# rst-tu-dortmund/teb_local_planner

Hardware: AMD Instinct MI355X
Metric: TEB LM iterations/sec (whole node) (higher is better)
Workload: dtype f64; 1 GPU; C4: 256 candidate TEBs/GPU x 200 poses at the start (teb_autosize on, the reference default: 193..287 poses, mean 234, after the step), 500 point obstacles (50 dynamic), diff-drive, point footprint, TebConfig defaults, 4 outer x 5 inner; tebs_per_gpu=256, tebs_total=256, poses=200, pose_capacity=288, tebs_ok=256, obstacles=500, jacobian_mode=analytic (closed form), exchange=none (single GPU), binary_hash=10be306ab42698fd, binary_variant_defines=

## Files before the change

include/teb_amd.h:

```cpp
#ifndef TEB_AMD_H_
#define TEB_AMD_H_

#include <stdint.h>

#ifdef __cplusplus
extern "C" {
#endif

#define TEB_AMD_ABI_VERSION 3
#define TEB_AMD_MAX_POSES 944

enum {
  TEB_AMD_OK = 0,
  TEB_AMD_ERR_INVALID_ARG = 1,
  TEB_AMD_ERR_NO_DEVICE = 2,
  TEB_AMD_ERR_HIP = 3,
  TEB_AMD_ERR_CAPACITY = 4,
  TEB_AMD_ERR_UNSUPPORTED = 5
};

enum {
  TEB_AMD_TEB_OK = 0,
  TEB_AMD_TEB_FAILED = 1,
  TEB_AMD_TEB_NONFINITE = 2
// ... 147 lines not shown
       TEB_AMD_LAYOUT_BAND_HBM = 3 };
enum { TEB_AMD_HSIG3D_AUTO = 0, TEB_AMD_HSIG3D_WIDE = 1, TEB_AMD_HSIG3D_SMALL = 2 };
typedef struct teb_amd_options {
  int32_t struct_size;
  int32_t layout;
  int32_t fixed_layout;
  int32_t band_ldlt;
  int32_t generic_distance_path;
  int32_t hsig3d_kernel;
  int32_t no_near_cache;
  int32_t multi_cu;
  int32_t multi_cu_timeout_us;
  int32_t speculative_trials;
  int32_t generic_config_path;
  int32_t compile_for_config;
  int32_t reserved[4];
} teb_amd_options_t;
void teb_amd_options_default(teb_amd_options_t* opt);

int  teb_amd_create(const teb_amd_config_t* cfg, int32_t max_tebs, int32_t max_poses,
                    int32_t max_obstacles, int32_t max_obstacle_vertices, int32_t max_via_points,
                    int32_t device, void* stream, teb_amd_handle_t** out);
int  teb_amd_create_ex(const teb_amd_config_t* cfg, int32_t max_tebs, int32_t max_poses,
                       int32_t max_obstacles, int32_t max_obstacle_vertices, int32_t max_via_points,
                       int32_t device, void* stream, const teb_amd_options_t* options, teb_amd_handle_t** out);
void teb_amd_destroy(teb_amd_handle_t* h);
int  teb_amd_set_config(teb_amd_handle_t* h, const teb_amd_config_t* cfg);

int  teb_amd_set_obstacles(teb_amd_handle_t* h, const teb_amd_obstacles_t* obst);
int  teb_amd_set_via_points(teb_amd_handle_t* h, int32_t count, const double* x, const double* y);

// ... 124 lines not shown
```

include/teb_amd_debug.h:

```cpp
#ifndef TEB_AMD_DEBUG_H_
#define TEB_AMD_DEBUG_H_
#include "teb_amd.h"
#ifdef __cplusplus
extern "C" {
#endif

int teb_amd_sizeof_config(void);
int teb_amd_sizeof_obstacles(void);
int teb_amd_sizeof_teb_batch(void);
int teb_amd_sizeof_results(void);
int teb_amd_sizeof_options(void);

int teb_amd_debug_linearize(teb_amd_handle_t* h, int32_t b, double weight_multiplier, double* H_dense,
                            double* bvec, double* chi2, int32_t* assoc_pose, int32_t* assoc_obst,
                            int32_t assoc_cap, int32_t* assoc_count);

int teb_amd_debug_distance(teb_amd_handle_t* h, int32_t nq, const int32_t* obst_index, const double* x,
                           const double* y, const double* theta, const int32_t* spatio_temporal,
                           const double* t, double* dist, double* grad);

int teb_amd_debug_profile(teb_amd_handle_t* h, double* cycles8);
int teb_amd_debug_profile_bands(teb_amd_handle_t* h, double* cycles_per_band);

int teb_amd_debug_stream(teb_amd_handle_t* h, int64_t n_doubles, int32_t repeats);
// ... 10 lines not shown
int teb_amd_debug_last_config_profile(teb_amd_handle_t* h, int32_t* defaults_profile);
int teb_amd_debug_last_instantiation(teb_amd_handle_t* h, int32_t* solver, int32_t* jacobian_mode, int32_t* scene_kind);
int teb_amd_debug_rtc_stats(int32_t* ready, int32_t* compiling, int32_t* failed, double* last_compile_seconds, char* last_error, int32_t capacity);
int teb_amd_debug_rtc_join(void);
int teb_amd_debug_rtc_compile(uint64_t flag_values, int32_t solver, int32_t jacobian_mode, int32_t scene_kind, int64_t* code_bytes);
int teb_amd_debug_rtc_cache(int32_t* embedded, int32_t* disk_hits, int32_t* disk_writes, char* cache_dir, int32_t capacity);

int teb_amd_debug_build_info(char* kernel_hash, int32_t kernel_hash_capacity, char* source_hash, int32_t source_hash_capacity, char* variant_defines,
                             int32_t defines_capacity, int32_t* threads_per_workgroup);

#define TEB_AMD_PHASE_LOG_SLOTS 9
int teb_amd_set_phase_log(teb_amd_handle_t* h, int32_t enable);
int teb_amd_get_phase_log(teb_amd_handle_t* h, double* cycles, int32_t capacity_bands, int32_t* bands);

int teb_amd_debug_assoc_overflow(teb_amd_handle_t* h, int32_t* flags);

#ifdef __cplusplus
}
#endif
#endif
```

teb_local_planner_amd/_abi.py:

```python
import ctypes as C

import numpy as np

MAX_FOOTPRINT_VERTICES = 64

OK, ERR_INVALID_ARG, ERR_NO_DEVICE, ERR_HIP, ERR_CAPACITY, ERR_UNSUPPORTED = range(6)
MAX_POSES = 944
TEB_OK, TEB_FAILED, TEB_NONFINITE = range(3)
FOOTPRINT_POINT, FOOTPRINT_CIRCULAR, FOOTPRINT_TWO_CIRCLES, FOOTPRINT_LINE, FOOTPRINT_POLYGON = range(5)
OBST_POINT, OBST_CIRCULAR, OBST_LINE, OBST_PILL, OBST_POLYGON = range(5)
ROT_LEFT, ROT_NONE, ROT_RIGHT = range(3)
JACOBIAN_ANALYTIC, JACOBIAN_G2O_NUMERIC = range(2)

c_i32 = C.c_int32
c_f64 = C.c_double
p_i32 = C.POINTER(C.c_int32)
p_f64 = C.POINTER(C.c_double)


class Config(C.Structure):
    _fields_ = [
        ("teb_autosize", c_i32), ("dt_ref", c_f64), ("dt_hysteresis", c_f64),
        ("min_samples", c_i32), ("max_samples", c_i32), ("exact_arc_length", c_i32),
        ("via_points_ordered", c_i32),
# ... 54 lines not shown
        ("max_number_classes", c_i32), ("max_number_plans_in_current_class", c_i32), ("h_signature_prescaler", c_f64),
        ("h_signature_threshold", c_f64), ("allow_init_with_backwards_motion", c_i32), ("delete_detours_backwards", c_i32),
        ("detours_orientation_tolerance", c_f64), ("length_start_orientation_vector", c_f64),
        ("max_ratio_detours_duration_best_duration", c_f64), ("global_plan_overwrite_orientation", c_i32),
        ("viapoints_all_candidates", c_i32),
    ]


LAYOUT_AUTO, LAYOUT_BLOCKS_LDS, LAYOUT_BAND_LDS, LAYOUT_BAND_HBM = 0, 1, 2, 3
HSIG3D_AUTO, HSIG3D_WIDE, HSIG3D_SMALL = 0, 1, 2


class Options(C.Structure):
    _fields_ = [("struct_size", c_i32), ("layout", c_i32), ("fixed_layout", c_i32), ("band_ldlt", c_i32),
                ("generic_distance_path", c_i32), ("hsig3d_kernel", c_i32), ("no_near_cache", c_i32), ("multi_cu", c_i32),
                ("multi_cu_timeout_us", c_i32), ("speculative_trials", c_i32), ("generic_config_path", c_i32), ("compile_for_config", c_i32), ("reserved", c_i32 * 4)]

    def __init__(self, layout=LAYOUT_AUTO, fixed_layout=False, band_ldlt=False, generic_distance_path=False, hsig3d_kernel=HSIG3D_AUTO,
                 no_near_cache=False, multi_cu=0, multi_cu_timeout_us=0, speculative_trials=0, generic_config_path=False, compile_for_config=0):
        super().__init__()
        self.struct_size = C.sizeof(Options)
        self.layout = {"auto": LAYOUT_AUTO, "cr": LAYOUT_BLOCKS_LDS, "band": LAYOUT_BAND_LDS, "bandg": LAYOUT_BAND_HBM}.get(layout, layout)
        self.fixed_layout = int(fixed_layout)
        self.band_ldlt = int(band_ldlt)
        self.generic_distance_path = int(generic_distance_path)
        self.hsig3d_kernel = {"auto": HSIG3D_AUTO, "wide": HSIG3D_WIDE, "small": HSIG3D_SMALL}.get(hsig3d_kernel, hsig3d_kernel)
        self.no_near_cache = int(no_near_cache)
        self.multi_cu = int(multi_cu)
        self.multi_cu_timeout_us = int(multi_cu_timeout_us)
        self.speculative_trials = int(speculative_trials)
        self.generic_config_path = int(generic_config_path)
        self.compile_for_config = int(compile_for_config)


class Results(C.Structure):
    _fields_ = [
        ("status", p_i32), ("lm_iterations", p_i32), ("lm_trials", p_i32), ("chi2", p_f64),
        ("cost", p_f64), ("lambda_", p_f64),
    ]


def _ptr(a, ty):
    if a is None:
        return C.cast(None, C.POINTER(ty))
    return a.ctypes.data_as(C.POINTER(ty))


# ... 191 lines not shown
```

teb_local_planner_amd/csrc/teb_amd.hip:

```cpp
#include <hip/hip_runtime.h>

#include <chrono>
#include <cmath>
#include <cstdio>
#include <unistd.h>
#include <cstdlib>
#include <algorithm>
#include <cstring>
#include <limits>
#include <string>
#include <random>
#include <vector>

#include "../../include/teb_amd.h"
#include "../../include/teb_amd_debug.h"
#define TEB_AMD_MAIN_TU
#include "teb_kernel.hpp"
#include "teb_opt_launch.hpp"
#include "teb_fleet.hpp"
#include "teb_strip.hpp"
#include "teb_hsig.hpp"
#include "teb_graph.hpp"
#include "teb_comm.hpp"
#include "teb_rtc.hpp"
// ... 686 lines not shown
  const size_t assoc_bytes = sizeof(int) * (size_t)max_tebs * max_poses * (size_t)(max_obstacles > 0 ? max_obstacles : 1);
  if (assoc_bytes > ((size_t)64 << 30)) return fail(TEB_AMD_ERR_CAPACITY, "association table would exceed 64 GiB");

  teb_amd_handle* h = new teb_amd_handle();
  h->device = device;
  h->cfg = *cfg;
  h->opt = opt;
  h->max_tebs = max_tebs; h->stride = max_poses; h->max_obst = max_obstacles; h->max_verts = max_obstacle_vertices;
  h->max_via = max_via_points;
  h->lds_bytes = lds;
  h->solver = solver; h->solver_created = solver;
  h->lds_limit = lds_limit;
  h->num_cus = prop.multiProcessorCount;
  h->plan = make_lds_plan(max_poses, solver, 0, h->lds_limit);
  h->hmat_stride = std::max(hbm_scratch_doubles(max_poses, SOLVER_BAND), hbm_scratch_doubles(max_poses, solver));
  h->hmat_stride = (h->hmat_stride + 1) & ~(size_t)1;
  h->band_ldlt = opt.band_ldlt != 0;
  if (solver == SOLVER_BANDG) h->band_ldlt = 0;
  if (stream) { h->stream = reinterpret_cast<hipStream_t>(stream); h->own_stream = false; }
  else {
    if (hipStreamCreateWithFlags(&h->stream, hipStreamNonBlocking) != hipSuccess) { delete h; return fail(TEB_AMD_ERR_HIP, "hipStreamCreate failed"); }
    h->own_stream = true;
  }
  const size_t BS = (size_t)max_tebs * max_poses;
  const size_t Mo = max_obstacles > 0 ? max_obstacles : 1;
  bool ok = true;
  auto A = [&](hipError_t e) { if (e != hipSuccess) ok = false; };
  A(h->o_type.alloc(Mo)); A(h->o_dyn.alloc(Mo)); A(h->o_voff.alloc(Mo + 1)); A(h->o_static.alloc(Mo)); A(h->o_dynidx.alloc(Mo));
  A(h->o_list.alloc(5 * (size_t)Mo));
  A(h->o_ax.alloc(Mo)); A(h->o_ay.alloc(Mo)); A(h->o_bx.alloc(Mo)); A(h->o_by.alloc(Mo)); A(h->o_rad.alloc(Mo));
  A(h->o_vx.alloc(Mo)); A(h->o_vy.alloc(Mo)); A(h->o_cx.alloc(Mo)); A(h->o_cy.alloc(Mo)); A(h->o_brad.alloc(Mo));
  A(h->o_pvx.alloc(max_obstacle_vertices)); A(h->o_pvy.alloc(max_obstacle_vertices));
  A(h->viax.alloc(max_via_points)); A(h->viay.alloc(max_via_points));
  A(h->n.alloc(max_tebs)); A(h->has_vs.alloc(max_tebs)); A(h->has_vg.alloc(max_tebs)); A(h->rotdir.alloc(max_tebs));
  A(h->via_en.alloc(max_tebs)); A(h->status.alloc(max_tebs)); A(h->optimized.alloc(max_tebs)); A(h->iters.alloc(max_tebs)); A(h->last_iters.alloc(max_tebs)); A(h->trials.alloc(max_tebs));
  A(h->assoc_cnt.alloc(BS)); A(h->assoc.alloc(BS * Mo)); A(h->assoc_ovf.alloc(max_tebs)); A(h->legacy_idx.alloc((size_t)max_tebs * Mo));
  A(h->via_pose.alloc((size_t)max_tebs * (max_via_points > 0 ? max_via_points : 1)));
  A(h->x.alloc(BS)); A(h->y.alloc(BS)); A(h->th.alloc(BS)); A(h->dt.alloc(BS));
  A(h->vs.alloc(3 * (size_t)max_tebs)); A(h->vg.alloc(3 * (size_t)max_tebs));
  A(h->chi2.alloc(max_tebs)); A(h->cost.alloc(max_tebs)); A(h->lambda.alloc(max_tebs));
  A(h->Hbackup.alloc((size_t)max_tebs * h->hmat_stride));
  A(h->clk.alloc(4));
  h->hband_stride = solver == SOLVER_BANDG ? (((size_t)hbo(4 * max_poses) + 2 + 1) & ~(size_t)1) : 0;
  A(h->Hband.alloc((size_t)max_tebs * h->hband_stride));
  A(h->snap_n.alloc(max_tebs)); A(h->snap_x.alloc(BS)); A(h->snap_y.alloc(BS)); A(h->snap_th.alloc(BS)); A(h->snap_dt.alloc(BS));
  A(h->dbg_H.alloc((size_t)4 * max_poses * kBand)); A(h->dbg_b.alloc((size_t)4 * max_poses)); A(h->dbg_chi2.alloc(4));
  A(h->sel_cost.alloc(2)); A(h->sel_idx.alloc(1)); A(h->err_flag.alloc(1));
  A(h->pack_dev.alloc(kPackMaxDoubles));
  if (ok && hipHostMalloc(reinterpret_cast<void**>(&h->pack_host), kPackMaxDoubles * sizeof(double), hipHostMallocDefault) != hipSuccess) h->pack_host = nullptr;
  A(h->stage_x.alloc((size_t)max_poses + 2)); A(h->stage_y.alloc((size_t)max_poses + 2)); A(h->stage_yaw.alloc((size_t)max_poses + 2));
  A(h->out_cmd.alloc(4 * (size_t)max_tebs)); A(h->out_prof.alloc((size_t)max_tebs * (max_poses + 1) * 3)); A(h->out_traj.alloc(BS * 7));
  A(h->hsig.alloc((size_t)max_tebs * (Mo > 2 ? Mo : 2))); A(h->hs_pre.alloc(Mo)); A(h->hs_pim.alloc(Mo)); A(h->hs_pex.alloc(Mo));
  if (ok && hipEventCreate(&h->ev0) != hipSuccess) ok = false;
  if (ok && hipEventCreate(&h->ev1) != hipSuccess) ok = false;
  for (int sv : {SOLVER_BAND, SOLVER_CR, SOLVER_BANDG})
    for (int jm : {TEB_AMD_JACOBIAN_ANALYTIC, TEB_AMD_JACOBIAN_G2O_NUMERIC})
// ... 569 lines not shown
#ifndef TEB_AMD_HAS_FLEET_UNITS
    return fail(TEB_AMD_ERR_UNSUPPORTED, "fleet launches exist in the product library only; this one is the variant built with [" TEB_AMD_VARIANT_DEFINES "]");
#else
    if (h->cfg.jacobian_mode != TEB_AMD_JACOBIAN_ANALYTIC)
      return fail(TEB_AMD_ERR_INVALID_ARG, "fleet launches need jacobian_mode TEB_AMD_JACOBIAN_ANALYTIC");
    for (int b = 0; b < h->B; ++b)
      if (h->fleet.band_scene[b] >= h->fleet.n_scenes) {
        char buf[160];
        std::snprintf(buf, sizeof buf, "band %d maps to scene %d, but %d scenes are set (teb_amd_set_band_scenes)", b, h->fleet.band_scene[b], h->fleet.n_scenes);
        return fail(TEB_AMD_ERR_INVALID_ARG, buf);
      }
#endif
  }
  OptArgs a;
  std::memset(&a, 0, sizeof a);
  a.inner = inner; a.outer = outer; a.compute_cost = compute_cost; a.no_near_cache = h->opt.no_near_cache != 0; a.band_ldlt = (fleet ? h->fleet.solver : h->solver) == SOLVER_BANDG ? 0 : h->band_ldlt; a.Hband = h->Hband.p; a.hband_stride = h->hband_stride;
  a.obst_scale = obst_cost_scale; a.via_scale = viapoint_cost_scale; a.alt_time = alternative_time_cost;
  if (h->iter_log_on) { a.iter_log = h->iter_log.p; a.iter_log_cap = TEB_AMD_ITERATION_LOG_ROWS; }
  if (h->phase_log_on) a.phase_log = h->phase_log.p;
#ifdef TEB_PROFILE
  a.dbg_H = h->dbg_H.p;
#endif
  h->last_inner = inner;
  return launch(h, a);
}

int teb_amd_set_iteration_log(teb_amd_handle_t* h, int32_t enable) {
  int rc = check_handle(h);
  if (rc) return rc;
  if (enable && !h->iter_log.p) {
    const size_t count = (size_t)h->max_tebs * TEB_AMD_ITERATION_LOG_ROWS * 4;
// ... 1386 lines not shown
    int S = kThreads * kPoseIterBandHbm;
    while (S > 2 && lds_bytes_for(S, SOLVER_BANDG, h->lds_limit) > h->lds_limit) --S;
    *max_poses_supported = S;
  }
  return TEB_AMD_OK;
}

int teb_amd_debug_linearize(teb_amd_handle_t* h, int32_t b, double weight_multiplier, double* H_dense, double* bvec,
                            double* chi2, int32_t* assoc_pose, int32_t* assoc_obst, int32_t assoc_cap, int32_t* assoc_count) {
  int rc = check_handle(h);
  if (rc) return rc;
  if ((rc = refuse_in_fleet_mode(h, "teb_amd_debug_linearize"))) return rc;
  if (b < 0 || b >= h->B) return fail(TEB_AMD_ERR_INVALID_ARG, "TEB index out of range");
  OptArgs a;
  std::memset(&a, 0, sizeof a);
  a.inner = 1; a.outer = 1; a.no_near_cache = h->opt.no_near_cache != 0; a.debug_linearize = 1; a.debug_weight_multiplier = weight_multiplier; a.band_ldlt = h->solver == SOLVER_BANDG ? 0 : h->band_ldlt; a.Hband = h->Hband.p; a.hband_stride = h->hband_stride;
  a.dbg_H = h->dbg_H.p; a.dbg_b = h->dbg_b.p; a.dbg_chi2 = h->dbg_chi2.p;
  SceneDev sc = scene_of(h);
  BatchDev bt = batch_of(h);
  const size_t so = (size_t)b * h->stride;
  bt.B = 1;
  bt.n += b; bt.x += so; bt.y += so; bt.th += so; bt.dt += so;
  bt.has_vs += b; bt.vs += 3 * b; bt.has_vg += b; bt.vg += 3 * b; bt.rotdir += b; bt.via_en += b;
  bt.status += b; bt.iters += b; bt.last_iters += b; bt.trials += b; bt.chi2 += b; bt.cost += b; bt.lambda += b;
  bt.assoc_cnt += so; bt.assoc += (size_t)b * bt.assoc_cap * h->stride; bt.assoc_overflow += b;
  bt.via_pose += (size_t)b * bt.via_cap; bt.Hbackup += (size_t)b * h->hmat_stride;
  int sv_i[3]; double sv_d[3];
  HIPCHK(hipMemcpy(&sv_i[0], h->status.p + b, sizeof(int), hipMemcpyDeviceToHost));
  HIPCHK(hipMemcpy(&sv_i[1], h->iters.p + b, sizeof(int), hipMemcpyDeviceToHost));
  HIPCHK(hipMemcpy(&sv_i[2], h->trials.p + b, sizeof(int), hipMemcpyDeviceToHost));
  HIPCHK(hipMemcpy(&sv_d[0], h->chi2.p + b, sizeof(double), hipMemcpyDeviceToHost));
// ... 273 lines not shown
  int rc = check_handle(h);
  if (rc) return rc;
  if (!defaults_profile) return fail(TEB_AMD_ERR_INVALID_ARG, "null output");
  *defaults_profile = h->last_defaults_profile;
  return TEB_AMD_OK;
}

int teb_amd_debug_mcu_flags(teb_amd_handle_t* h, int32_t flags) {
  int rc = check_handle(h);
  if (rc) return rc;
  h->mcu_debug_flags = flags;
  return TEB_AMD_OK;
}


int teb_amd_debug_assoc_overflow(teb_amd_handle_t* h, int32_t* flags) {
  int rc = check_handle(h);
  if (rc) return rc;
  HIPCHK(hipMemcpy(flags, h->assoc_ovf.p, h->B * sizeof(int), hipMemcpyDeviceToHost));
  return TEB_AMD_OK;
}

}
```

teb_local_planner_amd/csrc/teb_device.hpp:

```cpp
#pragma once
#include <hip/hip_runtime.h>
#include <stdint.h>

#include "../../include/teb_amd.h"

#define TEB_PF_ALL(X)                                                                                                              \
  X(EXACT_ARC) X(COST_EXPONENT) X(NEW_ASSOCIATION) X(DYNAMIC_EDGES) X(VIA_POINTS) X(NONHOLONOMIC_VELOCITY) X(VELOCITY_EDGES)      \
  X(ACCELERATION_EDGES) X(NONHOLONOMIC_ACCELERATION) X(TIME_OPTIMAL) X(SHORTEST_PATH) X(VELOCITY_OBSTACLE_RATIO) X(RADIUS_FREE)   \
  X(DEBUG_LINEARIZE) X(BAND_LDLT) X(INFLATED) X(NO_NEAR_CACHE) X(DIVERGENCE_DETECTION) X(KIN_DIFF_DRIVE) X(KIN_EDGES)
#define TEB_PF_EXPR_EXACT_ARC (c.exact_arc_length)
#define TEB_PF_DFLT_EXACT_ARC false
#define TEB_PF_EXPR_COST_EXPONENT (c.obstacle_cost_exponent != 1.0 && c.min_obstacle_dist > 0.0)
#define TEB_PF_DFLT_COST_EXPONENT false
#define TEB_PF_EXPR_NEW_ASSOCIATION (!c.legacy_obstacle_association)
#define TEB_PF_DFLT_NEW_ASSOCIATION true
#define TEB_PF_EXPR_DYNAMIC_EDGES (c.include_dynamic_obstacles && c.weight_obstacle != 0)
#define TEB_PF_DFLT_DYNAMIC_EDGES true
#define TEB_PF_HOST_DYNAMIC_EDGES (c.weight_obstacle != 0)
#define TEB_PF_EXPR_VIA_POINTS (sc.nvia > 0 && c.weight_viapoint != 0)
#define TEB_PF_DFLT_VIA_POINTS false
#define TEB_PF_WIDE_VIA_POINTS 1
#define TEB_PF_EXPR_NONHOLONOMIC_VELOCITY (c.max_vel_y == 0)
#define TEB_PF_DFLT_NONHOLONOMIC_VELOCITY true
#define TEB_PF_WIDE_NONHOLONOMIC_VELOCITY 1
// ... 208 lines not shown
  size_t hmat_stride;
  long long* clk;
};

struct OptArgs {
  int inner, outer, compute_cost;
  double obst_scale, via_scale;
  int alt_time;
  double* Hband;
  size_t hband_stride;
  int band_ldlt;
  int no_near_cache;
  double* iter_log;
  int iter_log_cap;
  int debug_linearize;
  double debug_weight_multiplier;
  double* dbg_H;
  double* dbg_b;
  double* dbg_chi2;
  double* phase_log;
};
constexpr int kPhaseLogSlots = 9;

}
```

teb_local_planner_amd/csrc/teb_kernel.hpp:

```cpp
#pragma once
#include "teb_edges.hpp"
#include "teb_multicu.hpp"
#include "teb_autoresize_chain.hpp"

namespace tebamd {

#ifdef TEB_PROFILE
#define PROF_DECL long long prof_t0 = 0, prof_wg_t0 = clock64(), prof_acc[8] = {0, 0, 0, 0, 0, 0, 0, 0};
#define PROF_START() prof_t0 = clock64()
#define PROF_END(k) prof_acc[k] += clock64() - prof_t0
#else
#define PROF_DECL const bool plog_ = args.phase_log != nullptr; long long* const plog_acc_ = reinterpret_cast<long long*>(l.red + 40); \
  if (plog_ && threadIdx.x == 0) { for (int q_ = 0; q_ < 9; ++q_) plog_acc_[q_] = 0; plog_acc_[9] = clock64(); }
#define PROF_START() do { if (plog_ && threadIdx.x == 0) plog_acc_[8] = clock64(); } while (0)
#define PROF_END(k) do { if (plog_ && threadIdx.x == 0) plog_acc_[k] += clock64() - plog_acc_[8]; } while (0)
#endif

#ifdef TEB_PROFILE
__device__ long long g_ev_prof[8];
#define EVP_DECL long long evp_t0 = clock64(), evp_t1;
#define EVP(k) do { __builtin_amdgcn_sched_barrier(0); asm volatile("s_waitcnt vmcnt(0) lgkmcnt(0)" ::: "memory"); evp_t1 = clock64(); __builtin_amdgcn_sched_barrier(0); if (blockIdx.x == 0 && threadIdx.x == 1) g_ev_prof[k] += evp_t1 - evp_t0; evp_t0 = evp_t1; } while (0)
__device__ unsigned long long g_assoc_stats[4];
__device__ unsigned long long g_ar_steps[4];
__device__ unsigned long long g_near_recomputed, g_near_queries;
// ... 31 lines not shown

__host__ __device__ inline int nb_for(int S) { return (4 * S + 7) / 8; }
constexpr size_t kLdsHeadroomBytes = 1024;
__host__ __device__ inline size_t hmat_doubles(int S, int solver) {
  if (solver == SOLVER_BANDG) return (size_t)6 * S + 256;
  if (solver == SOLVER_CR) return (size_t)nb_for(S) * (2 * kBlk + 8);
  const size_t band = (size_t)hbo(4 * S), compact = (size_t)((nb_for(S) + 1) / 2) * (2 * kBlk + 8) + 14;
  return ((band > compact ? band : compact) + 1) & ~(size_t)1;
}
__host__ __device__ inline size_t hbm_scratch_doubles(int S, int solver) {
  const size_t nb = (size_t)nb_for(S);
  const size_t blocks = nb * (2 * kBlk + 8);
  const size_t own = hmat_doubles(S, solver);
  return own > blocks ? own : blocks;
}
__host__ inline LdsPlan make_lds_plan(int S, int solver, int ob_entries, size_t lds_limit_bytes) {
  LdsPlan p;
  p.S = S; p.solver = solver;
  int o = 0;
  p.off_state = o; o += 7 * S;
  o = (o + 1) & ~1;
  int hm = (int)hmat_doubles(S, solver);
  if (solver == SOLVER_BANDG) {
    const long long room = (long long)(lds_limit_bytes / 8) - (o + 8LL * S + 16 + 96 + 5LL * (ob_entries > 0 ? ob_entries : 0)), want = 64LL * 2 * kBlk;
    const long long extra = (room < want ? room : want) & ~1LL;
    if (extra > hm) hm = (int)extra;
  }
  p.off_H = o; o += hm;
  p.off_b = o; o += 4 * S + 8;
  p.off_dx = o; o += 4 * S + 8;
// ... 93 lines not shown
  return bi;
}

struct TebCtx {
  int b, n;
  int has_vs, has_vg, rotdir, via_en;
  double vs[3], vg[3];
  double w_obst;
  bool inflated;
  const int* assoc_cnt;
  const int* assoc;
  const int* via_pose;
  int stride;
  int assoc_cap;
  McuView mcu;
};

__device__ __forceinline__ double footprint_bound_radius(const teb_amd_config_t& c) {
  double frad = 0;
  if (c.footprint_type == TEB_AMD_FOOTPRINT_CIRCULAR) frad = c.footprint_radius;
  else if (c.footprint_type == TEB_AMD_FOOTPRINT_TWO_CIRCLES)
    frad = fmax(fabs(c.footprint_front_offset) + c.footprint_front_radius, fabs(c.footprint_rear_offset) + c.footprint_rear_radius);
  else if (c.footprint_type == TEB_AMD_FOOTPRINT_LINE || c.footprint_type == TEB_AMD_FOOTPRINT_POLYGON)
    for (int v = 0; v < c.footprint_n_vertices; ++v) frad = fmax(frad, sqrt(c.footprint_vx[v] * c.footprint_vx[v] + c.footprint_vy[v] * c.footprint_vy[v]));
  return frad;
}
__device__ __forceinline__ double distance_lower_bound(const SceneDev& sc, int oi, double x, double y, double frad) {
  const double bx = sc.cx[oi] - x, by = sc.cy[oi] - y;
  const double lbd = sqrt(bx * bx + by * by) - sc.brad[oi] - frad;
  return lbd - 1e-9 * (fabs(lbd) + sc.brad[oi] + frad + 1.0);
// ... 60 lines not shown
  if (uncached || __any(!(ddx * ddx + ddy * ddy <= lim * lim))) {
    int d_lo, d_hi;
    dyn_chunk(sc, sl, nsl, d_lo, d_hi);
    mask = dyn_near_mask<MODE>(c, sc, l, i, d_lo, d_lo + 64 < d_hi ? d_lo + 64 : d_hi, m);
    if (pass == 0) { nc.m0 = mask; nc.rx0 = x; nc.ry0 = y; } else if (!(kMaxPoseIter > 2 && pass >= 2)) { nc.m1 = mask; nc.rx1 = x; nc.ry1 = y; }
#ifdef TEB_PROFILE
    atomicAdd(&g_near_recomputed, 1ull);
#endif
  }
#ifdef TEB_PROFILE
  atomicAdd(&g_near_queries, 1ull);
#endif
  return mask;
}

template <int MODE, bool FAST, int PART = 0>
__device__ __forceinline__ void eval_index(const teb_amd_config_t& c, const SceneDev& sc, const TebCtx& t,
                                           const Lds& l, int i, Accum& A, unsigned long long near_first, int sl = 0, int nsl = 1) {
  constexpr bool JAC = (MODE == 1);
  const int n = t.n;
  const bool first = (sl == 0);
  int d_lo, d_hi;
  dyn_chunk(sc, sl, nsl, d_lo, d_hi);
  Win w;
  w.x0 = l.sx[i]; w.y0 = l.sy[i]; w.t0 = l.sth[i]; w.d0 = l.sdt[i];
  w.x1 = l.sx[i + 1]; w.y1 = l.sy[i + 1]; w.t1 = l.sth[i + 1];
  w.c0 = l.cs[i]; w.s0 = l.sn[i]; w.c1 = l.cs[i + 1]; w.s1 = l.sn[i + 1];
  const bool has2 = (i + 2 <= n - 1);
  w.d1 = has2 ? l.sdt[i + 1] : 1.0;
  w.x2 = has2 ? l.sx[i + 2] : 0.0; w.y2 = has2 ? l.sy[i + 2] : 0.0; w.t2 = has2 ? l.sth[i + 2] : 0.0;
  const bool seg_active = (n > 2);

  int pre[4] = {0, 0, 0, 0};
  if constexpr (FAST && MODE != 2) {
    if (i >= 1 && TEB_CFGI(NEW_ASSOCIATION)) {
#pragma unroll
      for (int u = 0; u < 4; ++u) {
        const int kq = sl + u * nsl;
        pre[u] = kq < t.assoc_cap ? t.assoc[(size_t)kq * t.stride + i] : 0;
      }
    }
  }
  const int cnt = FAST ? t.assoc_cnt[i] : ld_list(t.mcu.shared_lists, t.assoc_cnt + i);
  EVP_DECL
  if (i >= 1) {
   if constexpr (PART != 2) {
    TEB_IF_FAST(FAST) {
      if (TEB_CFGI(NEW_ASSOCIATION)) {
        constexpr int kStaticBatch = 4;
        if constexpr (MODE == 2) {
          for (int k = sl; k < cnt; k += nsl) {
            const int p = t.assoc[(size_t)k * t.stride + i];
            const double ox = l.obx[p], oy = l.oby[p], orad = l.obr[p];
            TEB_EDGE(M_POSE0, CAT_OBST, edge_obstacle_fast<J_>(c, ox, oy, orad, W, t.w_obst, t.inflated, ACC_));
          }
        } else {
          int cur[kStaticBatch];
#pragma unroll
          for (int u = 0; u < kStaticBatch; ++u) cur[u] = pre[u];
          for (int k0 = sl; k0 < cnt; k0 += kStaticBatch * nsl) {
            int pp[kStaticBatch];
            bool valid[kStaticBatch];
#pragma unroll
            for (int u = 0; u < kStaticBatch; ++u) {
              const int kq = k0 + u * nsl;
              valid[u] = kq < cnt;
              pp[u] = valid[u] ? cur[u] : 0;
              const int kn = kq + kStaticBatch * nsl;
              cur[u] = kn < cnt ? t.assoc[(size_t)kn * t.stride + i] : 0;
// ... 211 lines not shown
  typedef const double __attribute__((address_space(1))) gdouble_t;
  typedef const teb_v2d __attribute__((address_space(1))) gv2d_t;
  for (int q = 2 * (int)threadIdx.x; q < hsz; q += 2 * kThreads)
    *reinterpret_cast<teb_v2d*>(hmat_ptr<SOLVER>(l, q, Nt)) = *reinterpret_cast<gv2d_t*>((gdouble_t*)g + q);
}

template <int SOLVER>
__device__ __forceinline__ double* diag_ptr(const Lds& l, int r) {
  return SOLVER != SOLVER_CR ? &l.Hb[hbo(r)] : &l.Db[(r >> 3) * kBlk + (r & 7) * 9];
}

__device__ __forceinline__ void refresh_trig(const Lds& l, int n) {
  for (int i = threadIdx.x; i < n; i += kThreads) { double sv, cv; sincos(l.sth[i], &sv, &cv); l.cs[i] = cv; l.sn[i] = sv; }
}

template <int SOLVER, int JMODE, bool FAST>
__device__ inline void linearize(const teb_amd_config_t& c, const SceneDev& sc, const TebCtx& t, const Lds& l, NearCache& nc,
                                 double* cats , bool trig_is_current = false) {
  const int n = t.n, Nt = 4 * n, tid = threadIdx.x;
  const int hsz = (SOLVER != SOLVER_CR) ? hbo(Nt) : ((Nt + 7) >> 3) * 2 * kBlk;
  LNP_DECL
  if constexpr (SOLVER != SOLVER_CR) {
    for (int q = 2 * tid; q < hsz; q += 2 * kThreads) *reinterpret_cast<teb_v2d*>(l.Hb + q) = teb_v2d{0.0, 0.0};
  } else {
    const int half = ((Nt + 7) >> 3) * kBlk;
    for (int q = 2 * tid; q < half; q += 2 * kThreads) {
      *reinterpret_cast<teb_v2d*>(l.Db + q) = teb_v2d{0.0, 0.0};
      *reinterpret_cast<teb_v2d*>(l.Lb + q) = teb_v2d{0.0, 0.0};
    }
  }
  for (int q = 2 * tid; q < Nt + 8; q += 2 * kThreads) *reinterpret_cast<teb_v2d*>(l.bv + q) = teb_v2d{0.0, 0.0};
  LNP(0);
  if (!trig_is_current) refresh_trig(l, n);
  __syncthreads();
  LNP(1);
  Accum A;
  A.clear_chi();
  for (int k0 = 0, pass = 0; k0 < n - 1; ++pass) {
    const int G = (k0 > 0 || kThreads > 256) ? lanes_per_pose(n - 1 - k0) : 1;
    const int i = k0 + tid / G, sl = tid % G;
    const bool active = i <= n - 2;
    constexpr int EM = JMODE == TEB_AMD_JACOBIAN_G2O_NUMERIC ? 2 : 1;
    const unsigned long long near = active ? dyn_near_cached<EM, FAST>(c, sc, l, i, sl, G, nc, pass) : 0ull;
    LNP(2);
    A.clear();
    if (active) eval_index<EM, FAST>(c, sc, t, l, i, A, near, sl, G);
    LNP(3);
    if (G > 1) {
      for (int off = 1; off < G; off <<= 1) {
#pragma unroll
        for (int q = 0; q < 6; ++q) A.H[q] += __shfl_xor(A.H[q], off, 64);
#pragma unroll
        for (int q = 0; q < 3; ++q) A.g[q] += __shfl_xor(A.g[q], off, 64);
      }
    }
    LNP(4);
    if (active && sl == 0) scatter<SOLVER, 0>(A, l, i, n);
    __syncthreads();
    if (active && sl == 0) scatter<SOLVER, 1>(A, l, i, n);
    __syncthreads();
    if (active && sl == 0) scatter<SOLVER, 2>(A, l, i, n);
    __syncthreads();
    LNP(5);
    k0 += kThreads / G;
  }
  if (tid < 3) { *diag_ptr<SOLVER>(l, tid) = 1.0; l.bv[tid] = 0; }
  if (tid >= 4 && tid < 8) { int r = 4 * (n - 1) + (tid - 4); *diag_ptr<SOLVER>(l, r) = 1.0; l.bv[r] = 0; }
  if (SOLVER == SOLVER_CR && tid >= 8 && tid < 12 && (n & 1)) {
    int r = 4 * n + (tid - 8); *diag_ptr<SOLVER>(l, r) = 1.0;
  }
  cats[0] = A.chi[0]; cats[1] = A.chi[1]; cats[2] = A.chi[2]; cats[3] = A.chi[3];
  block_sum<4>(cats, l.red);
  LNP(6);
}

template <bool FAST, int PART>
__device__ __forceinline__ void evaluate_pass(const teb_amd_config_t& c, const SceneDev& sc, const TebCtx& t, const Lds& l, NearCache& nc, Accum& A) {
  for (int k0 = 0, pass = 0; k0 < t.n - 1; ++pass) {
    const int G = (k0 > 0 || kThreads > 256) ? lanes_per_pose(t.n - 1 - k0) : 1;
    const int i = k0 + (int)threadIdx.x / G;
    if (i <= t.n - 2) {
      const unsigned long long near = dyn_near_cached<0, FAST>(c, sc, l, i, (int)threadIdx.x % G, G, nc, pass);
      eval_index<0, FAST, PART>(c, sc, t, l, i, A, near, (int)threadIdx.x % G, G);
    }
    k0 += kThreads / G;
  }
}
template <bool FAST>
__device__ inline void evaluate(const teb_amd_config_t& c, const SceneDev& sc, const TebCtx& t, const Lds& l, NearCache& nc,
                                double* cats , bool trig_is_current = false) {
  if (!trig_is_current) {
    refresh_trig(l, t.n);
    __syncthreads();
  }
  Accum A;
  A.clear_chi();
  evaluate_pass<FAST, 0>(c, sc, t, l, nc, A);
  cats[0] = A.chi[0]; cats[1] = A.chi[1]; cats[2] = A.chi[2]; cats[3] = A.chi[3];
  block_sum<5>(cats, l.red);
}
__device__ inline bool evaluate_mcu(const teb_amd_config_t& c, const SceneDev& sc, const TebCtx& t, const Lds& l, NearCache& nc, McuMaster& m, int S,
                                    double* cats ) {
  refresh_trig(l, t.n);
  __syncthreads();
  mcu_publish(m, l.sx, l.sy, l.cs, l.sn, l.tdyn, t.n, S);
  mcu_issue(m, MCU_KIND_DIST, t.n);
  Accum A;
  A.clear_chi();
  const bool overlap = c.weight_velocity_obstacle_ratio == 0;
  if (overlap) evaluate_pass<false, 2>(c, sc, t, l, nc, A);
  const bool ok = mcu_wait(m, l.ired + 26);
  if (ok) {
// ... 2031 lines not shown
          }
          index = block_argmin(best, bi, l.red, l.ired);
          if (index == 0x7fffffff) index = -1;
        }
        if (c.via_points_ordered) start_pose_idx = index + 2;
        if (index > n - 2) index = n - 2;
        int attach = index;
        if (index < 1) attach = c.via_points_ordered ? 1 : -1;
        if (tid == 0) via_pose[v] = attach;
      }
    } else {
      for (int v = tid; v < sc.nvia; v += kThreads) via_pose[v] = -1;
    }
    __threadfence_block();
    __syncthreads();
    LNP(11);
    PROF_END(1);

    near_cache.invalidate();
    if (args.inner <= 0 && !TEB_CFGI(DEBUG_LINEARIZE)) { status = TEB_AMD_TEB_FAILED; break; }
    t.mcu.items = nullptr;
    if (mcu_on && obst_edges && !(mc.debug_flags & 2)) {
      mcu_publish(mm, l.sx, l.sy, l.cs, l.sn, l.tdyn, n, S);
      mcu_issue(mm, MCU_KIND_DIST, n);
      if (!mcu_wait(mm, l.ired + 26)) { status = TEB_AMD_TEB_FAILED; if (tid == 0) or_agent_i32(bt.assoc_overflow + b, 4); break; }
      t.mcu.items = mcu_items;
    }
    double ni = 2;
    bool lm_ok = true;
    last_iters = 0;
// ... 233 lines not shown
```

teb_local_planner_amd/planner.py:

```python
import ctypes as C
import os

import numpy as np

from . import _abi
from .config import TebConfig

_HERE = os.path.dirname(os.path.abspath(__file__))
_LIB = None


class TebAmdError(RuntimeError):
    def __init__(self, code, what, msg):
        super().__init__("%s failed: status %d (%s)" % (what, code, msg))
        self.code = code


def lib():
    global _LIB
    if _LIB is None:
        so = os.environ.get("TEB_AMD_LIB") or os.path.join(_HERE, "libteb_amd.so")
        if not os.path.exists(so):
            raise TebAmdError(-1, "load", "libteb_amd.so missing: run `python -m teb_local_planner_amd.build`")
        L = C.CDLL(so)
# ... 23 lines not shown
            L.teb_amd_multi_cu_backoff.argtypes = [vp, _abi.p_i32, _abi.p_i32]
        if hasattr(L, "teb_amd_set_iteration_log"):
            L.teb_amd_set_iteration_log.argtypes = [vp, C.c_int32]
            L.teb_amd_get_iteration_log.argtypes = [vp, C.c_int32, _abi.p_f64, C.c_int32, _abi.p_i32]
            L.teb_amd_debug_world_argmin.argtypes = [_abi.p_f64, C.c_int32, _abi.p_i32, _abi.p_f64, _abi.p_i32]
        L.teb_amd_device_state.argtypes = [vp] + [C.POINTER(vp)] * 5 + [_abi.p_i32]
        L.teb_amd_snapshot_state.argtypes = [vp]
        L.teb_amd_restore_state.argtypes = [vp]
        L.teb_amd_last_kernel_ms.argtypes = [vp, C.POINTER(C.c_float)]
        L.teb_amd_capacity.argtypes = [vp, _abi.p_i32, _abi.p_i32]
        L.teb_amd_debug_linearize.argtypes = [vp, C.c_int32, C.c_double, _abi.p_f64, _abi.p_f64, _abi.p_f64,
                                              _abi.p_i32, _abi.p_i32, C.c_int32, _abi.p_i32]
        L.teb_amd_debug_distance.argtypes = [vp, C.c_int32, _abi.p_i32, _abi.p_f64, _abi.p_f64, _abi.p_f64,
                                             _abi.p_i32, _abi.p_f64, _abi.p_f64, _abi.p_f64]
        L.teb_amd_debug_assoc_overflow.argtypes = [vp, _abi.p_i32]
        L.teb_amd_debug_stream.argtypes = [vp, C.c_int64, C.c_int32]
        L.teb_amd_debug_profile.argtypes = [vp, _abi.p_f64]
        d, i32 = C.c_double, C.c_int32
        L.teb_amd_init_trajectory_line.argtypes = [vp, i32, _abi.p_f64, _abi.p_f64, d, d, i32, i32]
        L.teb_amd_init_trajectory_plan.argtypes = [vp, i32, i32, _abi.p_f64, _abi.p_f64, _abi.p_f64, d, d, i32, i32, i32]
        L.teb_amd_init_trajectory_path.argtypes = [vp, i32, i32, _abi.p_f64, _abi.p_f64, d, d, _abi.p_f64, _abi.p_f64, _abi.p_f64,
                                                   i32, i32]
        L.teb_amd_update_and_prune.argtypes = [vp, i32, _abi.p_f64, _abi.p_f64, i32]
        L.teb_amd_set_velocity_start.argtypes = [vp, i32, i32, _abi.p_f64]
        L.teb_amd_set_velocity_goal.argtypes = [vp, i32, i32, _abi.p_f64]
        L.teb_amd_get_pose_counts.argtypes = [vp, _abi.p_i32, _abi.p_i32]
        L.teb_amd_get_velocity_command.argtypes = [vp, i32, i32, i32, _abi.p_f64, _abi.p_f64, _abi.p_f64, _abi.p_i32]
        L.teb_amd_get_velocity_profile.argtypes = [vp, i32, _abi.p_f64, i32, _abi.p_i32]
        L.teb_amd_get_full_trajectory.argtypes = [vp, i32, _abi.p_f64, i32, _abi.p_i32]
        L.teb_amd_has_diverged.argtypes = [vp, i32, _abi.p_i32]
# ... 471 lines not shown
        _chk(lib().teb_amd_debug_distance(self._h, nq, _abi._ptr(oi, C.c_int32), _abi._ptr(x, C.c_double),
                                          _abi._ptr(y, C.c_double), _abi._ptr(th, C.c_double),
                                          _abi._ptr(st, C.c_int32), _abi._ptr(tt, C.c_double),
                                          _abi._ptr(d, C.c_double), _abi._ptr(g, C.c_double)),
             "teb_amd_debug_distance")
        return d, g

    def debug_stream(self, n_doubles, repeats=1):
        _chk(lib().teb_amd_debug_stream(self._h, int(n_doubles), int(repeats)), "teb_amd_debug_stream")

    def debug_overflow_flags(self):
        f = np.zeros(self.count, np.int32)
        _chk(lib().teb_amd_debug_assoc_overflow(self._h, _abi._ptr(f, C.c_int32)), "debug_assoc_overflow")
        return f


def make_solver(cfg, obst, via, batch, device=0, stream=None, max_tebs=None, max_poses=None, options=None):
    nverts = len(obst.vert_x)
    s = TebBatchSolver(cfg, max_tebs or batch.count, max_poses or batch.stride, max(len(obst), 1), max(nverts, 1),
                       max(len(via), 1), device=device, stream=stream, options=options)
    s.set_obstacles(obst)
    s.set_via_points(via)
    s.upload(batch)
    return s


class TebOptimalPlanner:

    def __init__(self, cfg, obstacles=None, via_points=None, max_poses=None, device=0):
        self.cfg_ = cfg
# ... 362 lines not shown
```

Measured before the change: 2.541 million TEB.LM-iterations/s.

## Load-balance static obstacle distance evaluation via flattened pose-obstacle item table

After obstacle association, each block prefix-scans the per-pose association counts and builds a flat table of (pose, obstacle) items in HBM scratch. Distances and gradients for all items are then computed evenly across all threads into LDS scratch (the H buffer region) before edge accumulation, instead of each pose's thread looping over its own varying obstacle count. Because the records occupy the H area, H zeroing moves to after the first pass reads them, which adds extra barriers. This aims to remove warp divergence and load imbalance from uneven association counts, at the cost of an extra pass, more LDS and global traffic, and synchronisation.

```diff
diff --git a/include/teb_amd.h b/include/teb_amd.h
--- a/include/teb_amd.h
+++ b/include/teb_amd.h
@@ -185,7 +185,8 @@
   int32_t speculative_trials;
   int32_t generic_config_path;
   int32_t compile_for_config;
-  int32_t reserved[4];
+  int32_t no_balanced_obstacle_edges;
+  int32_t reserved[3];
 } teb_amd_options_t;
 void teb_amd_options_default(teb_amd_options_t* opt);
 
diff --git a/include/teb_amd_debug.h b/include/teb_amd_debug.h
--- a/include/teb_amd_debug.h
+++ b/include/teb_amd_debug.h
@@ -48,6 +48,7 @@
 int teb_amd_get_phase_log(teb_amd_handle_t* h, double* cycles, int32_t capacity_bands, int32_t* bands);
 
 int teb_amd_debug_assoc_overflow(teb_amd_handle_t* h, int32_t* flags);
+int teb_amd_debug_balanced_items(teb_amd_handle_t* h, int32_t band, int32_t* in_use, int32_t* counted);
 
 #ifdef __cplusplus
 }
diff --git a/teb_local_planner_amd/_abi.py b/teb_local_planner_amd/_abi.py
--- a/teb_local_planner_amd/_abi.py
+++ b/teb_local_planner_amd/_abi.py
@@ -92,10 +92,12 @@
 class Options(C.Structure):
     _fields_ = [("struct_size", c_i32), ("layout", c_i32), ("fixed_layout", c_i32), ("band_ldlt", c_i32),
                 ("generic_distance_path", c_i32), ("hsig3d_kernel", c_i32), ("no_near_cache", c_i32), ("multi_cu", c_i32),
-                ("multi_cu_timeout_us", c_i32), ("speculative_trials", c_i32), ("generic_config_path", c_i32), ("compile_for_config", c_i32), ("reserved", c_i32 * 4)]
+                ("multi_cu_timeout_us", c_i32), ("speculative_trials", c_i32), ("generic_config_path", c_i32), ("compile_for_config", c_i32),
+                ("no_balanced_obstacle_edges", c_i32), ("reserved", c_i32 * 3)]
 
     def __init__(self, layout=LAYOUT_AUTO, fixed_layout=False, band_ldlt=False, generic_distance_path=False, hsig3d_kernel=HSIG3D_AUTO,
-                 no_near_cache=False, multi_cu=0, multi_cu_timeout_us=0, speculative_trials=0, generic_config_path=False, compile_for_config=0):
+                 no_near_cache=False, multi_cu=0, multi_cu_timeout_us=0, speculative_trials=0, generic_config_path=False, compile_for_config=0,
+                 no_balanced_obstacle_edges=False):
         super().__init__()
         self.struct_size = C.sizeof(Options)
         self.layout = {"auto": LAYOUT_AUTO, "cr": LAYOUT_BLOCKS_LDS, "band": LAYOUT_BAND_LDS, "bandg": LAYOUT_BAND_HBM}.get(layout, layout)
@@ -109,6 +111,7 @@
         self.speculative_trials = int(speculative_trials)
         self.generic_config_path = int(generic_config_path)
         self.compile_for_config = int(compile_for_config)
+        self.no_balanced_obstacle_edges = int(no_balanced_obstacle_edges)
 
 
 class Results(C.Structure):
diff --git a/teb_local_planner_amd/csrc/teb_amd.hip b/teb_local_planner_amd/csrc/teb_amd.hip
--- a/teb_local_planner_amd/csrc/teb_amd.hip
+++ b/teb_local_planner_amd/csrc/teb_amd.hip
@@ -724,6 +724,7 @@
   h->num_cus = prop.multiProcessorCount;
   h->plan = make_lds_plan(max_poses, solver, 0, h->lds_limit);
   h->hmat_stride = std::max(hbm_scratch_doubles(max_poses, SOLVER_BAND), hbm_scratch_doubles(max_poses, solver));
+  h->hmat_stride += flat_tail_doubles(max_poses);
   h->hmat_stride = (h->hmat_stride + 1) & ~(size_t)1;
   h->band_ldlt = opt.band_ldlt != 0;
   if (solver == SOLVER_BANDG) h->band_ldlt = 0;
@@ -750,6 +751,7 @@
   A(h->vs.alloc(3 * (size_t)max_tebs)); A(h->vg.alloc(3 * (size_t)max_tebs));
   A(h->chi2.alloc(max_tebs)); A(h->cost.alloc(max_tebs)); A(h->lambda.alloc(max_tebs));
   A(h->Hbackup.alloc((size_t)max_tebs * h->hmat_stride));
+  if (ok) A(hipMemset(h->Hbackup.p, 0, (size_t)max_tebs * h->hmat_stride * sizeof(double)));
   A(h->clk.alloc(4));
   h->hband_stride = solver == SOLVER_BANDG ? (((size_t)hbo(4 * max_poses) + 2 + 1) & ~(size_t)1) : 0;
   A(h->Hband.alloc((size_t)max_tebs * h->hband_stride));
@@ -1349,7 +1351,7 @@
   }
   OptArgs a;
   std::memset(&a, 0, sizeof a);
-  a.inner = inner; a.outer = outer; a.compute_cost = compute_cost; a.no_near_cache = h->opt.no_near_cache != 0; a.band_ldlt = (fleet ? h->fleet.solver : h->solver) == SOLVER_BANDG ? 0 : h->band_ldlt; a.Hband = h->Hband.p; a.hband_stride = h->hband_stride;
+  a.inner = inner; a.outer = outer; a.compute_cost = compute_cost; a.no_near_cache = h->opt.no_near_cache != 0; a.no_balanced_obstacle_edges = h->opt.no_balanced_obstacle_edges != 0; a.band_ldlt = (fleet ? h->fleet.solver : h->solver) == SOLVER_BANDG ? 0 : h->band_ldlt; a.Hband = h->Hband.p; a.hband_stride = h->hband_stride;
   a.obst_scale = obst_cost_scale; a.via_scale = viapoint_cost_scale; a.alt_time = alternative_time_cost;
   if (h->iter_log_on) { a.iter_log = h->iter_log.p; a.iter_log_cap = TEB_AMD_ITERATION_LOG_ROWS; }
   if (h->phase_log_on) a.phase_log = h->phase_log.p;
@@ -2766,7 +2768,7 @@
   if (b < 0 || b >= h->B) return fail(TEB_AMD_ERR_INVALID_ARG, "TEB index out of range");
   OptArgs a;
   std::memset(&a, 0, sizeof a);
-  a.inner = 1; a.outer = 1; a.no_near_cache = h->opt.no_near_cache != 0; a.debug_linearize = 1; a.debug_weight_multiplier = weight_multiplier; a.band_ldlt = h->solver == SOLVER_BANDG ? 0 : h->band_ldlt; a.Hband = h->Hband.p; a.hband_stride = h->hband_stride;
+  a.inner = 1; a.outer = 1; a.no_near_cache = h->opt.no_near_cache != 0; a.no_balanced_obstacle_edges = h->opt.no_balanced_obstacle_edges != 0; a.debug_linearize = 1; a.debug_weight_multiplier = weight_multiplier; a.band_ldlt = h->solver == SOLVER_BANDG ? 0 : h->band_ldlt; a.Hband = h->Hband.p; a.hband_stride = h->hband_stride;
   a.dbg_H = h->dbg_H.p; a.dbg_b = h->dbg_b.p; a.dbg_chi2 = h->dbg_chi2.p;
   SceneDev sc = scene_of(h);
   BatchDev bt = batch_of(h);
@@ -3070,6 +3072,18 @@
 }
 
 
+int teb_amd_debug_balanced_items(teb_amd_handle_t* h, int32_t band, int32_t* in_use, int32_t* counted) {
+  int rc = check_handle(h);
+  if (rc) return rc;
+  if (band < 0 || band >= h->max_tebs) return fail(TEB_AMD_ERR_INVALID_ARG, "teb_amd_debug_balanced_items: band out of range");
+  HIPCHK(hipStreamSynchronize(h->stream));
+  int32_t hdr[kFlatHeaderInts] = {0, 0};
+  HIPCHK(hipMemcpy(hdr, h->Hbackup.p + (size_t)(band + 1) * h->hmat_stride - flat_tail_doubles(h->stride), sizeof hdr, hipMemcpyDeviceToHost));
+  if (in_use) *in_use = hdr[0];
+  if (counted) *counted = hdr[1];
+  return TEB_AMD_OK;
+}
+
 int teb_amd_debug_assoc_overflow(teb_amd_handle_t* h, int32_t* flags) {
   int rc = check_handle(h);
   if (rc) return rc;
diff --git a/teb_local_planner_amd/csrc/teb_device.hpp b/teb_local_planner_amd/csrc/teb_device.hpp
--- a/teb_local_planner_amd/csrc/teb_device.hpp
+++ b/teb_local_planner_amd/csrc/teb_device.hpp
@@ -246,6 +246,7 @@
   double* iter_log;
   int iter_log_cap;
   int debug_linearize;
+  int no_balanced_obstacle_edges;
   double debug_weight_multiplier;
   double* dbg_H;
   double* dbg_b;
diff --git a/teb_local_planner_amd/csrc/teb_kernel.hpp b/teb_local_planner_amd/csrc/teb_kernel.hpp
--- a/teb_local_planner_amd/csrc/teb_kernel.hpp
+++ b/teb_local_planner_amd/csrc/teb_kernel.hpp
@@ -69,6 +69,11 @@
   const size_t own = hmat_doubles(S, solver);
   return own > blocks ? own : blocks;
 }
+constexpr int kFlatItemsPerPose = 8;
+constexpr int kFlatPoseShift = 20;
+constexpr int kFlatHeaderInts = 2;
+__host__ __device__ inline int flat_off_ints(int S) { return (S + 1) & ~1; }
+__host__ __device__ inline size_t flat_tail_doubles(int S) { return ((size_t)kFlatHeaderInts + flat_off_ints(S) + (size_t)kFlatItemsPerPose * S + 1) / 2; }
 __host__ inline LdsPlan make_lds_plan(int S, int solver, int ob_entries, size_t lds_limit_bytes) {
   LdsPlan p;
   p.S = S; p.solver = solver;
@@ -192,6 +197,9 @@
   int stride;
   int assoc_cap;
   McuView mcu;
+  int flat_total;
+  const int* flat_off;
+  const int* flat_tab;
 };
 
 __device__ __forceinline__ double footprint_bound_radius(const teb_amd_config_t& c) {
@@ -282,9 +290,44 @@
   return mask;
 }
 
+template <bool JAC, int W>
+__device__ __forceinline__ void flat_round(const teb_amd_config_t& c, const SceneDev& sc, const TebCtx& t, const Lds& l, double* rec, int q0) {
+  const int total = t.flat_total;
+  int it[W];
+#pragma unroll
+  for (int u = 0; u < W; ++u) {
+    const int q = q0 + u * kThreads;
+    it[u] = q < total ? t.flat_tab[q] : 0;
+  }
+  double dist[W], g0[W], g1[W];
+#pragma unroll
+  for (int u = 0; u < W; ++u) {
+    const int i = it[u] >> kFlatPoseShift, p = it[u] & ((1 << kFlatPoseShift) - 1);
+    double gr[2];
+    dist[u] = pointlike_distance<JAC>(c, l.sx[i], l.sy[i], l.obx[p], l.oby[p], TEB_CFGI(RADIUS_FREE) ? 0.0 : l.obr[p], gr);
+    g0[u] = JAC ? gr[0] : 0.0; g1[u] = JAC ? gr[1] : 0.0;
+  }
+#pragma unroll
+  for (int u = 0; u < W; ++u) {
+    const int q = q0 + u * kThreads;
+    if (q < total) {
+      rec[q] = dist[u];
+      if (JAC) { rec[total + q] = g0[u]; rec[2 * total + q] = g1[u]; }
+    }
+  }
+}
+template <bool JAC>
+__device__ __forceinline__ void flat_distances(const teb_amd_config_t& c, const SceneDev& sc, const TebCtx& t, const Lds& l) {
+  const int total = t.flat_total;
+  int q0 = threadIdx.x, wq = (int)threadIdx.x & ~63;
+  for (; wq + 3 * kThreads < total; q0 += 4 * kThreads, wq += 4 * kThreads) flat_round<JAC, 4>(c, sc, t, l, l.Db, q0);
+  for (; wq < total; q0 += 2 * kThreads, wq += 2 * kThreads) flat_round<JAC, 2>(c, sc, t, l, l.Db, q0);
+}
+
 template <int MODE, bool FAST, int PART = 0>
 __device__ __forceinline__ void eval_index(const teb_amd_config_t& c, const SceneDev& sc, const TebCtx& t,
-                                           const Lds& l, int i, Accum& A, unsigned long long near_first, int sl = 0, int nsl = 1) {
+                                           const Lds& l, int i, Accum& A, unsigned long long near_first, int sl = 0, int nsl = 1,
+                                           const double* flat_rec = nullptr ) {
   constexpr bool JAC = (MODE == 1);
   const int n = t.n;
   const bool first = (sl == 0);
@@ -300,8 +343,11 @@
   const bool seg_active = (n > 2);
 
   int pre[4] = {0, 0, 0, 0};
+  int flat_base = 0;
   if constexpr (FAST && MODE != 2) {
-    if (i >= 1 && TEB_CFGI(NEW_ASSOCIATION)) {
+    if (flat_rec != nullptr) {
+      if (i >= 1) flat_base = t.flat_off[i];
+    } else if (i >= 1 && TEB_CFGI(NEW_ASSOCIATION)) {
 #pragma unroll
       for (int u = 0; u < 4; ++u) {
         const int kq = sl + u * nsl;
@@ -321,6 +367,25 @@
             const int p = t.assoc[(size_t)k * t.stride + i];
             const double ox = l.obx[p], oy = l.oby[p], orad = l.obr[p];
             TEB_EDGE(M_POSE0, CAT_OBST, edge_obstacle_fast<J_>(c, ox, oy, orad, W, t.w_obst, t.inflated, ACC_));
+          }
+        } else if (flat_rec != nullptr) {
+          const int ftot = t.flat_total;
+          for (int k0 = 0; k0 < cnt; k0 += kStaticBatch) {
+            bool valid[kStaticBatch];
+            double dist[kStaticBatch], g0[kStaticBatch], g1[kStaticBatch];
+#pragma unroll
+            for (int u = 0; u < kStaticBatch; ++u) {
+              valid[u] = k0 + u < cnt;
+              const int q = valid[u] ? flat_base + k0 + u : 0;
+              dist[u] = flat_rec[q];
+              g0[u] = JAC ? flat_rec[ftot + q] : 0.0; g1[u] = JAC ? flat_rec[2 * ftot + q] : 0.0;
+            }
+#pragma unroll
+            for (int u = 0; u < kStaticBatch; ++u)
+              if (valid[u]) {
+                const double gr[2] = {g0[u], g1[u]};
+                obstacle_rows<JAC>(c, dist[u], gr, t.w_obst, t.inflated, A);
+              }
           }
         } else {
           int cur[kStaticBatch];
@@ -562,12 +627,9 @@
   for (int i = threadIdx.x; i < n; i += kThreads) { double sv, cv; sincos(l.sth[i], &sv, &cv); l.cs[i] = cv; l.sn[i] = sv; }
 }
 
-template <int SOLVER, int JMODE, bool FAST>
-__device__ inline void linearize(const teb_amd_config_t& c, const SceneDev& sc, const TebCtx& t, const Lds& l, NearCache& nc,
-                                 double* cats , bool trig_is_current = false) {
-  const int n = t.n, Nt = 4 * n, tid = threadIdx.x;
-  const int hsz = (SOLVER != SOLVER_CR) ? hbo(Nt) : ((Nt + 7) >> 3) * 2 * kBlk;
-  LNP_DECL
+template <int SOLVER>
+__device__ __forceinline__ void hmat_zero(const Lds& l, int hsz, int Nt) {
+  const int tid = threadIdx.x;
   if constexpr (SOLVER != SOLVER_CR) {
     for (int q = 2 * tid; q < hsz; q += 2 * kThreads) *reinterpret_cast<teb_v2d*>(l.Hb + q) = teb_v2d{0.0, 0.0};
   } else {
@@ -577,9 +639,24 @@
       *reinterpret_cast<teb_v2d*>(l.Lb + q) = teb_v2d{0.0, 0.0};
     }
   }
+}
+
+template <int SOLVER, int JMODE, bool FAST>
+__device__ inline void linearize(const teb_amd_config_t& c, const SceneDev& sc, const TebCtx& t, const Lds& l, NearCache& nc,
+                                 double* cats , bool trig_is_current = false) {
+  const int n = t.n, Nt = 4 * n, tid = threadIdx.x;
+  const int hsz = (SOLVER != SOLVER_CR) ? hbo(Nt) : ((Nt + 7) >> 3) * 2 * kBlk;
+  LNP_DECL
+  constexpr int EM = JMODE == TEB_AMD_JACOBIAN_G2O_NUMERIC ? 2 : 1;
+  bool flat = false;
+  if constexpr (FAST && EM != 2 && SOLVER != SOLVER_BANDG) flat = t.flat_total > 0;
+  if (!flat) hmat_zero<SOLVER>(l, hsz, Nt);
   for (int q = 2 * tid; q < Nt + 8; q += 2 * kThreads) *reinterpret_cast<teb_v2d*>(l.bv + q) = teb_v2d{0.0, 0.0};
   LNP(0);
   if (!trig_is_current) refresh_trig(l, n);
+  if constexpr (FAST && EM != 2 && SOLVER != SOLVER_BANDG) {
+    if (flat) flat_distances<true>(c, sc, t, l);
+  }
   __syncthreads();
   LNP(1);
   Accum A;
@@ -588,12 +665,17 @@
     const int G = (k0 > 0 || kThreads > 256) ? lanes_per_pose(n - 1 - k0) : 1;
     const int i = k0 + tid / G, sl = tid % G;
     const bool active = i <= n - 2;
-    constexpr int EM = JMODE == TEB_AMD_JACOBIAN_G2O_NUMERIC ? 2 : 1;
+    const bool use_rec = flat && k0 == 0;
     const unsigned long long near = active ? dyn_near_cached<EM, FAST>(c, sc, l, i, sl, G, nc, pass) : 0ull;
     LNP(2);
     A.clear();
-    if (active) eval_index<EM, FAST>(c, sc, t, l, i, A, near, sl, G);
+    if (active) eval_index<EM, FAST>(c, sc, t, l, i, A, near, sl, G, use_rec ? l.Db : nullptr);
     LNP(3);
+    if (use_rec) {
+      __syncthreads();
+      hmat_zero<SOLVER>(l, hsz, Nt);
+      __syncthreads();
+    }
     if (G > 1) {
       for (int off = 1; off < G; off <<= 1) {
 #pragma unroll
@@ -623,13 +705,14 @@
 }
 
 template <bool FAST, int PART>
-__device__ __forceinline__ void evaluate_pass(const teb_amd_config_t& c, const SceneDev& sc, const TebCtx& t, const Lds& l, NearCache& nc, Accum& A) {
+__device__ __forceinline__ void evaluate_pass(const teb_amd_config_t& c, const SceneDev& sc, const TebCtx& t, const Lds& l, NearCache& nc, Accum& A,
+                                              bool flat = false ) {
   for (int k0 = 0, pass = 0; k0 < t.n - 1; ++pass) {
     const int G = (k0 > 0 || kThreads > 256) ? lanes_per_pose(t.n - 1 - k0) : 1;
     const int i = k0 + (int)threadIdx.x / G;
     if (i <= t.n - 2) {
       const unsigned long long near = dyn_near_cached<0, FAST>(c, sc, l, i, (int)threadIdx.x % G, G, nc, pass);
-      eval_index<0, FAST, PART>(c, sc, t, l, i, A, near, (int)threadIdx.x % G, G);
+      eval_index<0, FAST, PART>(c, sc, t, l, i, A, near, (int)threadIdx.x % G, G, (flat && k0 == 0) ? l.Db : nullptr);
     }
     k0 += kThreads / G;
   }
@@ -641,9 +724,17 @@
     refresh_trig(l, t.n);
     __syncthreads();
   }
+  bool flat = false;
+  if constexpr (FAST) {
+    flat = t.flat_total > 0;
+    if (flat) {
+      flat_distances<false>(c, sc, t, l);
+      __syncthreads();
+    }
+  }
   Accum A;
   A.clear_chi();
-  evaluate_pass<FAST, 0>(c, sc, t, l, nc, A);
+  evaluate_pass<FAST, 0>(c, sc, t, l, nc, A, flat);
   cats[0] = A.chi[0]; cats[1] = A.chi[1]; cats[2] = A.chi[2]; cats[3] = A.chi[3];
   block_sum<5>(cats, l.red);
 }
@@ -2705,6 +2796,37 @@
     }
     __threadfence_block();
     __syncthreads();
+    t.flat_total = 0;
+    if constexpr (FAST && SOLVER != SOLVER_BANDG && JMODE == TEB_AMD_JACOBIAN_ANALYTIC) {
+      TEB_IF_FAST(FAST) {
+        int* const fhdr = reinterpret_cast<int*>(Hbk + bt.hmat_stride - flat_tail_doubles(S));
+        int* const foff = fhdr + kFlatHeaderInts;
+        int* const ftab = foff + flat_off_ints(S);
+        int* const scan = reinterpret_cast<int*>(l.Db);
+        const bool wanted = obst_edges && TEB_CFGI(NEW_ASSOCIATION) && args.no_balanced_obstacle_edges == 0;
+        const int lane = tid & 63, wv = tid >> 6;
+        const int my = (wanted && tid >= 1 && tid <= n - 2) ? assoc_cnt[tid] : 0;
+        int inc = my;
+#pragma unroll
+        for (int o = 1; o < 64; o <<= 1) { const int v = __shfl_up(inc, o, 64); if (lane >= o) inc += v; }
+        if (lane == 63) scan[wv] = inc;
+        __syncthreads();
+        int before = 0, total = 0;
+#pragma unroll
+        for (int w = 0; w < kWaves; ++w) { const int v = scan[w]; if (w < wv) before += v; total += v; }
+        total = uni_i(total);
+        const bool flat_ok = total > 0 && total <= kFlatItemsPerPose * S && 3 * total <= plan.off_b - plan.off_H && sc.n_static < (1 << kFlatPoseShift);
+        if (flat_ok) {
+          const int first = before + inc - my;
+          if (tid <= n - 2) foff[tid] = first;
+          for (int k = 0; k < my; ++k) ftab[first + k] = (tid << kFlatPoseShift) | assoc[(size_t)k * S + tid];
+          t.flat_total = total; t.flat_off = foff; t.flat_tab = ftab;
+        }
+        if (tid == 0) { fhdr[0] = flat_ok ? total : 0; fhdr[1] = total; }
+        __threadfence_block();
+        __syncthreads();
+      }
+    }
     LNP(11);
     PROF_END(1);
 
diff --git a/teb_local_planner_amd/planner.py b/teb_local_planner_amd/planner.py
--- a/teb_local_planner_amd/planner.py
+++ b/teb_local_planner_amd/planner.py
@@ -61,6 +61,8 @@
         L.teb_amd_debug_distance.argtypes = [vp, C.c_int32, _abi.p_i32, _abi.p_f64, _abi.p_f64, _abi.p_f64,
                                              _abi.p_i32, _abi.p_f64, _abi.p_f64, _abi.p_f64]
         L.teb_amd_debug_assoc_overflow.argtypes = [vp, _abi.p_i32]
+        if hasattr(L, "teb_amd_debug_balanced_items"):
+            L.teb_amd_debug_balanced_items.argtypes = [vp, C.c_int32, _abi.p_i32, _abi.p_i32]
         L.teb_amd_debug_stream.argtypes = [vp, C.c_int64, C.c_int32]
         L.teb_amd_debug_profile.argtypes = [vp, _abi.p_f64]
         d, i32 = C.c_double, C.c_int32
@@ -562,6 +564,11 @@
         _chk(lib().teb_amd_debug_assoc_overflow(self._h, _abi._ptr(f, C.c_int32)), "debug_assoc_overflow")
         return f
 
+    def debug_balanced_items(self, band=0):
+        a, b = C.c_int32(0), C.c_int32(0)
+        _chk(lib().teb_amd_debug_balanced_items(self._h, int(band), C.byref(a), C.byref(b)), "debug_balanced_items")
+        return a.value, b.value
+
 
 def make_solver(cfg, obst, via, batch, device=0, stream=None, max_tebs=None, max_poses=None, options=None):
     nverts = len(obst.vert_x)
```

Result: slower. 2.498 million TEB.LM-iterations/s (-1.7%).
